# modichirag/GSM-VI

Measured on AMD Instinct MI355X. Metric: GSM updates/sec at D=1024,B=32 (dense-cov gsm_update, fp64), higher is better.
Workload: dtype f64; 1 GPU; BASELINE configs[2]: D=1024 dense-cov Gaussian target, B=32, one GSM update per step; D=1024, B=32, instances=21, ring_bytes=352321536, launch=hipGraph(90 x 21 updates/replay + 1 x 7), warmup_steps_run=28, parallelism=single GPU

## Files before the change

### gsm-vi_amd/csrc/gsmvi_abi.hip

```cpp
#include <hip/hip_runtime.h>

#include <cstdio>
#include <cstdlib>
#include <cstring>
#include <string>

#include "../../include/gsmvi_hip.h"
#include "../../include/gsmvi_hip_debug.h"

void gsmvi_launch_panel_partial(hipStream_t st, hipEvent_t* ev, int MT, dim3 grid, int D, int ncols, int nrows,
                                const double* A, int lda, const double* shift, double alpha, const double* M,
                                int ldm, double* Pp, int chunks_per_wg, int a_vec_ok);
void gsmvi_launch_panel_finish(hipStream_t st, hipEvent_t* ev, int D, int nrows, int KC, const double* Pp,
                               const double* addvec, double* Out, int ldo, int ncols_out);
void gsmvi_launch_gsm_scalars(hipStream_t st, hipEvent_t* ev, int D, int B, int KC, const double* X, int ldx,
                              const double* G, int ldg, const double* mu0, const double* Pp, double* rec,
                              int ldrec);
size_t gsmvi_cov_update_lds_bytes(int SB);
hipError_t gsmvi_cov_update_prepare();
hipError_t gsmvi_bam_prepare();
hipError_t gsmvi_batched_prepare();
hipError_t gsmvi_bam_batched_prepare();
hipError_t gsmvi_psis_batched_prepare();
hipError_t gsmvi_psis_loo_batched_prepare();
// ... 4 lines not shown
                          const double* M, int ldm, int mrows, double* Pp, int* kc_out);
void gsmvi_launch_commit(hipStream_t st, int D, const int* info, const double* mu_new, const double* S_new,
                         int lds_new, double* mu, double* S, int lds, int* n_reverts);
void gsmvi_launch_panel_fast(hipStream_t st, hipEvent_t* ev, int MT, dim3 grid, int D, int nrows, const double* A,
                             int lda, const double* shift, double alpha, const double* M, int ldm, double* Pp,
                             int chunks_per_wg, int ncols, unsigned long long* stamps, double* Out, int ldo,
                             const double* addvec, const struct gsmvi_panel_extras* px);
bool gsmvi_launch_gsm_scalars_fast(hipStream_t st, hipEvent_t* ev, int D, int B, int KC, const double* X, int ldx,
                                   const double* G, int ldg, const double* mu0, const double* Pp, double* rec,
                                   int ldrec, int nt, unsigned long long* stamps);
bool gsmvi_launch_gsm_cov_sym(hipStream_t st, hipEvent_t* ev, int D, int B, const double* rec, int ldrec,
                              const double* mu0, const double* S0, int lds0, double* S, int lds, double* mu_out,
                              int dbg, unsigned long long* stamps, int num_cu);
void gsmvi_launch_panel_fast_part(hipStream_t st, hipEvent_t* ev, dim3 grid, int D, int B, const double* G, int ldg,
                                  const double* S0, int lds0, double* Pp, int chunks_per_wg, const double* X, int ldx,
                                  const double* mu0, double* Qg, double* Qm, int chw, unsigned long long* stamps);
void gsmvi_launch_gsm_cov_sym_slabs(hipStream_t st, hipEvent_t* ev, int D, int B, const struct gsm_slab_src& fs, const double* mu0,
                                    const double* S0, int lds0, double* S, int lds, double* mu_out, int kct, bool fold,
                                    unsigned long long* stamps);
int gsmvi_cov_sym_pairs(int nt);
int gsmvi_panel_fast_chunk(int MT);
int gsmvi_potrf_impl(struct gsmvi_ctx* ctx, hipStream_t st, int D, const double* S, int lds, double* R, int ldr,
                     int* info_dev);
int gsmvi_gram_impl(hipStream_t st, int D, const double* F, int ldf, double* C, int ldc, double shift, const double* shift_dev);
int gsmvi_whiten_impl(hipStream_t st, int D, int nrows, const double* R, int ldr, const double* X, int ldx,
                      const double* mu, double* Z, int ldz, double* logdiag);
int gsmvi_factor_impl(struct gsmvi_ctx* ctx, hipStream_t st, int D, int B, const double* Z, int ldz, const double* X,
                      int ldx, const double* G, int ldg, const double* mu0, const double* F0, int ldf0, double* mu,
                      double* F, int ldf, int* info_dev, int* n_reverts_dev);
int gsmvi_factor_local_impl(struct gsmvi_ctx* ctx, hipStream_t st, int D, int Bl, const double* Z, int ldz,
                            const double* X, int ldx, const double* G, int ldg, const double* mu0, const double* F0,
                            int ldf0, double* rec, int ldrec);
int gsmvi_factor_apply_impl(struct gsmvi_ctx* ctx, hipStream_t st, int D, int B, const double* Z, int ldz,
                            const double* rec, int ldrec, const double* mu0, const double* F0, int ldf0, double* mu,
// ... 230 lines not shown
    else if (!strcmp(name, "wide")) ctx->tune_wide = value;
    else if (!strcmp(name, "wide_kc")) ctx->tune_wide_kc = value;
    else if (!strcmp(name, "fork_min_D")) ctx->tune_fork_min_D = value;
    else if (!strcmp(name, "gram_mt")) ctx->tune_gram_mt = value > 0 ? value : 4;
    else if (!strcmp(name, "bam_full")) ctx->tune_bam_full = value;
    else if (!strcmp(name, "bam_kenq")) ctx->tune_bam_kenq = value;
    else if (!strcmp(name, "bam_hint_slack")) ctx->tune_bam_hint_slack = value;
    else if (!strcmp(name, "rider_direct_max_D")) ctx->tune_rider_direct_max_D = value;
    else if (!strcmp(name, "chain_pair")) ctx->tune_chain_pair = value;
    else if (!strcmp(name, "bam_batched_pad")) ctx->tune_bam_batched_pad = value;
    else if (!strcmp(name, "lowrank_kp")) ctx->tune_lowrank_kp = value;
    else if (!strcmp(name, "bam_basis")) ctx->tune_bam_basis = value;
    else if (!strcmp(name, "scalars_nt")) ctx->tune_scalars_nt = value;
    else if (!strcmp(name, "gsm_two_launch")) ctx->tune_gsm_two_launch = value;
    else if (!strcmp(name, "cov_fold_diag")) ctx->tune_cov_fold_diag = value;
    else if (!strcmp(name, "cov_dbg")) ctx->tune_cov_dbg = value;
    else if (!strcmp(name, "timeline")) {
        if (value && !ctx->stamps) {
            HIP_TRY(hipMalloc(reinterpret_cast<void**>(&ctx->stamps), GSMVI_STAMP_WORDS * sizeof(unsigned long long)));
            HIP_TRY(hipMemset(ctx->stamps, 0, GSMVI_STAMP_WORDS * sizeof(unsigned long long)));
        }
        ctx->tune_timeline = value;
    }
    else {
        gsmvi_set_error("%s: unknown tuning knob %s", __func__, name);
        return GSMVI_ERR_BAD_ARG;
    }
    return GSMVI_OK;
}

// ... 278 lines not shown
        *chw_out = 512;
    }
    return true;
}

static int gsm_two_launch(gsmvi_ctx* ctx, hipStream_t hs, int D, int B, int cpw, int kc, int chw, const double* X, int ldx,
                          const double* G, int ldg, const double* mu0, const double* S0, int lds0, double* mu, double* S,
                          int lds) {
    const int strips = D / 16;
    double* Qg = ctx->sg;
    double* Qm = Qg + (size_t)B * kc * strips;
    ctx->px = gsmvi_panel_extras();
    ctx->px_used = 1;
    hipEvent_t* ev0 = ctx->stage_events(0);
    ctx->ev_valid[1] = 0;
    gsmvi_launch_panel_fast_part(hs, ev0, dim3(strips, kc, chw == 512 ? B / 16 : 1), D, B, G, ldg, S0, lds0, ctx->pp, cpw, X, ldx, mu0, Qg, Qm, chw,
                                 ctx->timeline_stamps(0));
    ctx->path |= GSMVI_PATH_PANEL_FAST | (chw == 512 ? GSMVI_PATH_PANEL_CHUNK512 : 0u);
    int st = check_launch("k_panel_fast(partials)");
    if (st != GSMVI_OK) return st;
    gsm_slab_src fs;
    fs.X = X;
    fs.ldx = ldx;
    fs.Pp = ctx->pp;
    fs.Qg = Qg;
    fs.Qm = Qm;
    fs.KC = kc;
    fs.strips = strips;
    const bool fold = ctx->tune_cov_fold_diag >= 2 || (ctx->tune_cov_fold_diag == 1 && gsmvi_cov_sym_pairs(D / 32) >= ctx->num_cu);
    gsmvi_launch_gsm_cov_sym_slabs(hs, ctx->stage_events(2), D, B, fs, mu0, S0, lds0, S, lds, mu, chw == 512 ? 2 : 4, fold,
                                   ctx->timeline_stamps(2));
    ctx->path |= GSMVI_PATH_COV_SYM | GSMVI_PATH_GSM_TWO_LAUNCH | (fold ? GSMVI_PATH_COV_FOLD_DIAG : 0u);
    return check_launch("k_gsm_cov_sym(slabs)");
}

int gsmvi_gsm_update_f64(gsmvi_ctx* ctx, void* stream, int D, int B, const double* X, int ldx, const double* G,
                         int ldg, const double* mu0, const double* S0, int lds0, double* mu, double* S, int lds) {
    int st = check_common(ctx, D, B, __func__);
    if (st != GSMVI_OK) return st;
    BAD_ARG(!X || !G || !mu0 || !S0 || !mu || !S, "NULL array");
    BAD_ARG(ldx < D || ldg < D || lds0 < D || lds < D, "leading dimension smaller than D");
    BAD_ARG(S == S0 || mu == mu0, "outputs must not alias inputs");
    hipStream_t hs = reinterpret_cast<hipStream_t>(stream);
    const int ldrec = 3 * D + (D & 1);
    int cpw2 = 0, kc2 = 0, chw2 = 0;
    if (gsm_two_launch_gate(ctx, D, B, X, ldx, G, ldg, mu0, S0, lds0, S, lds, &cpw2, &kc2, &chw2))
        return gsm_two_launch(ctx, hs, D, B, cpw2, kc2, chw2, X, ldx, G, ldg, mu0, S0, lds0, mu, S, lds);
// ... 294 lines not shown
```

### gsm-vi_amd/csrc/gsmvi_ctx.h

```cpp
#pragma once
#include <hip/hip_runtime.h>
#include <cstddef>

#define GSMVI_MAX_KC 8
#define GSMVI_FACTOR_NMAX 256
#define GSMVI_STAMP_WORDS (4 * 4096)

struct gsmvi_panel_extras {
    const double* msl = nullptr;
    int kcm = 0;
    size_t mstride = 0;
    int ldsl = 0, msplit = 0;
    double* mfin = nullptr;
    int ldfin = 0;
    const double* sj_src = nullptr;
    int sj_kc = 0;
    size_t sj_stride = 0;
    int sj_len = 0;
    double* sj_dst = nullptr;
    int rd_on = 0, rd_n = 0, rd_B = 0, rd_kcg = 0, rd_jmode = 0;
    const double* rd_Gp = nullptr;
    double *rd_Kmat = nullptr, *rd_coef = nullptr;
    int* rd_bad = nullptr;
    unsigned long long* rd_stamps = nullptr;
// ... 52 lines not shown
    double* pp = nullptr;
    double* sg = nullptr;
    double *fo_Rt = nullptr, *fo_Tm = nullptr, *fo_Fs = nullptr;
    double* small = nullptr;
    int* ints = nullptr;
    double* gram_slabs = nullptr;
    int tune_panel_kc = 0;
    int tune_update_sb = 0;
    int tune_cov_dbg = 0;
    int tune_timeline = 0;
    unsigned long long* stamps = nullptr;
    int tune_direct_out = 1;
    int tune_scalars_nt = 0;
    int tune_no_fast = 0;
    int tune_cov_fold_diag = 1;
    int tune_gsm_two_launch = 1;
    int* bam_hint_host = nullptr;
    int tune_bam_kenq = 0;
    int tune_bam_hint_slack = 1;
    int tune_rider_direct_max_D = 2048;
    int tune_bam_full = 0;
    int tune_lowrank_kp = 0;
    int tune_bam_batched_pad = 1;
    int tune_chain_pair = 1;
    gsmf_bam_mean bam_mean = {nullptr, nullptr, {0.0, nullptr}};
    int bam_mean_done = 0;
    const double* chain_r11 = nullptr;
    const double* chain_w11 = nullptr;
    const double* reg_dev = nullptr;
    int tune_bam_basis = 1;
// ... 50 lines not shown
```

### gsm-vi_amd/csrc/gsmvi_fast.hip

```cpp
#include "gsmvi_common.h"
#include "gsmvi_ctx.h"
#include "gsmvi_small16.h"
#include <hip/hip_ext.h>

#define GSMVI_LAUNCH(kern, grid, block, shmem, st, ev, ...)                                         \
    do {                                                                                           \
        if (ev)                                                                                    \
            hipExtLaunchKernelGGL(kern, grid, block, shmem, st, (ev)[0], (ev)[1], 0, __VA_ARGS__); \
        else                                                                                       \
            hipLaunchKernelGGL(kern, grid, block, shmem, st, __VA_ARGS__);                         \
    } while (0)

template <int MT, bool HAS_SHIFT, int CHW, bool EXTRA, bool RIDER = false, bool RAG = false, bool PART = false>
__global__ __launch_bounds__(512) void k_panel_fast(int D, int nrows, const double* __restrict__ A, int lda,
                                                    const double* __restrict__ shift, double alpha,
                                                    const double* __restrict__ M, int ldm,
                                                    double* Pp, int chunks_per_wg, int ncols,
                                                    unsigned long long* __restrict__ stamps, double* __restrict__ Out,
                                                    int ldo, const double* __restrict__ addvec, gsmvi_panel_extras px) {
#define PSTAMP(k)                                                                                              \
    do {                                                                                                       \
        const unsigned wg_ = (blockIdx.z * gridDim.y + blockIdx.y) * gridDim.x + blockIdx.x;                   \
        if (stamps && threadIdx.x == 0 && wg_ < GSMVI_STAMP_WG)                                                \
            stamps[(size_t)wg_ * 8 + (k)] = __builtin_amdgcn_s_memrealtime();                                  \
    } while (0)
    PSTAMP(0);
    constexpr int LDG = CHW + 2;
    constexpr int NR = 16 * MT;
// ... 7 lines not shown
    if (RIDER && blockIdx.x == gridDim.x - 1) {
        if (blockIdx.y == 0 && blockIdx.z == 0)
            gsmf_small16_body(As, px.rd_n, px.rd_B, px.rd_Gp, px.rd_kcg, px.rd_Kmat, px.rd_coef, px.rd_bad, px.rd_stamps,
                              px.rd_jmode, px.rd_prior, px.rd_Pi, px.rd_R11, px.rd_W11);
        return;
    }
    const int tid = threadIdx.x, w = tid >> 6, l = tid & 63, c = l & 15, ks = l >> 4;
    const int jx = blockIdx.x * 16 + c;
    const int j = (RAG && jx >= ncols) ? ncols - 1 : jx;
    const int r0 = blockIdx.z * NR;

    v4d acc[MT];
#pragma unroll
    for (int mt = 0; mt < MT; ++mt) acc[mt] = (v4d){0.0, 0.0, 0.0, 0.0};
    static_assert(!PART || (MT <= 2 && !RAG && !RIDER && !HAS_SHIFT), "partial dots: one pass of the store loop, on the grid");
    double pq_g = 0.0, pq_x = 0.0, pq_m = 0.0;

    for (int ch = 0; ch < chunks_per_wg; ++ch) {
        const int cbase = (blockIdx.y * chunks_per_wg + ch) * CHW;
        if (cbase >= D) break;
        const int wbase = cbase + w * RW;
        const bool wave_in = wbase < D;
        v2d ga[UPT];
        v2d gs[UPT];
        unsigned okbits = 0;
#pragma unroll
        for (int q = 0; q < UPT; ++q) {
            const int u = q * 512 + tid;
            const int row = u / U16, c16 = u % U16;
            const int grow = r0 + row;
            const int col = cbase + 2 * c16;
// ... 44 lines not shown
        } else if (!RAG || wbase + RW <= D) {
            const double* mp = M + (size_t)((wave_in ? wbase : 0) + ks) * ldm + j;
#pragma unroll
            for (int s = 0; s < NST; ++s) m[s] = mp[(size_t)(4 * s) * ldm];
        } else {
            const int rb = wave_in ? wbase : 0;
#pragma unroll
            for (int s = 0; s < NST; ++s) {
                const int r = rb + ks + 4 * s;
                m[s] = M[(size_t)(r < D ? r : D - 1) * ldm + j];
            }
        }
        if constexpr (PART) {
            const int prow = r0 + ((tid >> 4) & (NR - 1)), pcol = blockIdx.x * 16 + (tid & 15);
            pq_g = A[(size_t)prow * lda + pcol];
            pq_x = px.sj_src[(size_t)prow * px.sj_len + pcol];
            pq_m = px.msl[pcol];
        }
        __builtin_amdgcn_sched_barrier(0);
        if (ch > 0) __syncthreads();
#pragma unroll
        for (int q = 0; q < UPT; ++q) {
            const int u = q * 512 + tid;
            const int row = u / U16, c16 = u % U16;
            v2d v = ga[q];
            if (!((okbits >> q) & 1u)) v = HAS_SHIFT ? gs[q] : (v2d){0.0, 0.0};
            if (HAS_SHIFT) { v.x -= gs[q].x; v.y -= gs[q].y; }
            v.x *= alpha; v.y *= alpha;
            *reinterpret_cast<v2d*>(&As[row * LDG + 2 * c16]) = v;
        }
        __syncthreads();
        PSTAMP(1);
// ... 20 lines not shown
#pragma unroll
        for (int r = 0; r < 4; ++r) red[(w * NR + 16 * mt + ks + 4 * r) * 17 + c] = acc[mt][r];
    __syncthreads();
    for (int idx = tid; idx < NR * 16; idx += 512) {
        const int rr = idx >> 4, cc = idx & 15;
        const int row = r0 + rr;
        if (row < nrows && (!RAG || (int)blockIdx.x * 16 + cc < ncols)) {
            double s = 0.0;
#pragma unroll
            for (int ww = 0; ww < 8; ww += 2) s += red[(ww * NR + rr) * 17 + cc] + red[((ww + 1) * NR + rr) * 17 + cc];
            if (Out == nullptr) Pp[((size_t)blockIdx.y * nrows + row) * ncols + blockIdx.x * 16 + cc] = s;
            else Out[(size_t)row * ldo + blockIdx.x * 16 + cc] = s + (addvec ? addvec[blockIdx.x * 16 + cc] : 0.0);
            if constexpr (PART) {
                const double pg = row16_sum(pq_g * s);
                if (cc == 0) px.sj_dst[((size_t)row * gridDim.y + blockIdx.y) * gridDim.x + blockIdx.x] = pg;
                if (blockIdx.y == 0) {
                    const double pm = row16_sum((pq_m - pq_x) * pq_g);
                    if (cc == 0) px.mfin[(size_t)row * gridDim.x + blockIdx.x] = pm;
                }
            }
        }
    }
    if (EXTRA && px.sj_src != nullptr) {
        const int nwg = gridDim.x * gridDim.y * gridDim.z;
        const int wg = (blockIdx.z * gridDim.y + blockIdx.y) * gridDim.x + blockIdx.x;
        const int per = (px.sj_len + nwg - 1) / nwg;
        const int i_end = (wg + 1) * per < px.sj_len ? (wg + 1) * per : px.sj_len;
        for (int i = wg * per + tid; i < i_end; i += (int)blockDim.x) {
            double t[GSMVI_MAX_KC];
#pragma unroll
            for (int q = 0; q < GSMVI_MAX_KC; ++q) t[q] = px.sj_src[(size_t)(q < px.sj_kc ? q : px.sj_kc - 1) * px.sj_stride + i];
            double a = 0.0;
#pragma unroll
            for (int q = 0; q < GSMVI_MAX_KC; ++q) a += (q < px.sj_kc) ? t[q] : 0.0;
// ... 159 lines not shown
    for (int e = 0; e < EPT; ++e) {
        const int i = tid + NT * e;
        if (i < D) {
            const double dmu = beta * ((sg[e] - dd[e]) - c * dd[e]);
            rb[i] = dd[e];
            rb[D + i] = dd[e] + dmu;
            rb[2 * D + i] = dmu;
        }
    }
    if (stamps) {
        asm volatile("s_waitcnt vmcnt(0)" ::: "memory");
        if (threadIdx.x == 0) stamps[(size_t)blockIdx.x * 8 + 3] = __builtin_amdgcn_s_memrealtime();
    }
}

template <int SB, bool RAG, bool FROM_SLABS = false, int KCT = 4, bool FOLD = false>
__global__ __launch_bounds__(512) __attribute__((amdgpu_waves_per_eu(FROM_SLABS ? 4 : 2))) void k_gsm_cov_sym(int D, int B, double invB, const double* __restrict__ rec, int ldrec,
                                                     const double* __restrict__ mu0,
                                                     const double* __restrict__ S0, int lds0,
                                                     double* __restrict__ S, int lds,
                                                     double* __restrict__ mu_out, int dbg,
                                                     unsigned long long* __restrict__ stamps, gsm_slab_src fs) {
    static_assert(!FOLD || FROM_SLABS, "folded diagonal tiles: the two-launch form only");
#define STAMP(k)                                                                          \
    do {                                                                                  \
        if (stamps && threadIdx.x == 0) stamps[(size_t)blockIdx.x * 8 + (k)] = __builtin_amdgcn_s_memrealtime(); \
    } while (0)
    if (blockIdx.x >= GSMVI_STAMP_WG) stamps = nullptr;
    STAMP(0);
    constexpr int RS = 48;
    constexpr int NPASS = (SB > 32) ? SB / 32 : 1;
    constexpr int SBP = SB / NPASS;
    constexpr int TILE = SBP * RS;
    constexpr int NU = SB * 16;
    constexpr int UPT = (6 * NU) / 512;
    static_assert((6 * NU) % 512 == 0, "tile units must divide over 512 threads");
    __shared__ __attribute__((aligned(16))) double smem[6 * TILE >= 2 * 32 * 33 ? 6 * TILE : 2 * 32 * 33];

// ... 18 lines not shown
        const int k = blockIdx.x - n_two;
        ti = ((nt & 1) ? 0 : 1) + 2 * k;
        tj0 = ti;
        two = false;
    }
    const bool diag = (tj0 == ti);
    const int I0 = ti * 32, J0 = tj0 * 32;
    const int tid = threadIdx.x, w = tid >> 6, l = tid & 63, c = l & 15, ks = l >> 4;
    const int t = w >> 2;
    const int wr = (w >> 1) & 1, wc = w & 1;
    const bool mine = (t == 0) || two;

    const int Jt = J0 + 32 * ((t == 1 && two) ? 1 : 0);
    const int tl = tid & 255;
    v2d s0v[2];
#pragma unroll
    for (int q = 0; q < 2; ++q) {
        const int unit = q * 256 + tl, i = unit >> 4, j2 = unit & 15;
        const int gr = (RAG && I0 + i >= D) ? D - 1 : I0 + i, gc = (RAG && Jt + 2 * j2 >= D) ? D - 2 : Jt + 2 * j2;
        s0v[q] = (dbg & 2) ? (v2d){1.0, 1.0} : *reinterpret_cast<const v2d*>(S0 + (size_t)gr * lds0 + gc);
    }
    const int X0 = (fold == 2) ? J0 + 32 : I0;
    v2d s0x = {0.0, 0.0};
    if constexpr (FOLD) {
        if (fold) s0x = *reinterpret_cast<const v2d*>(S0 + (size_t)(X0 + (tid >> 4)) * lds0 + X0 + 2 * (tid & 15));
    }
    __builtin_amdgcn_sched_barrier(0);
    v2d stg[UPT];
    double dmu_part = 0.0;
    v2d dmuI = {0.0, 0.0};
    v2d dmuX = {0.0, 0.0};
    if constexpr (FROM_SLABS) {
        static_assert(!RAG && NPASS == 1 && 512 % NU == 0, "two-launch form: B == SB in {16, 32}, on the grid");
        static_assert(KCT == 2 || KCT == 4, "slab count of the two-launch form");
        constexpr int NQG = 2 * KCT;
        const int u = tid & (NU - 1), b = u >> 4, ln = u & 15, c2 = 2 * ln;
        const bool st_d = (NU == 512) || tid < NU, st_e = (NU == 512) || tid >= NU;
        const int nqg = (fs.KC * fs.strips) >> 1, nqm = fs.strips >> 1;
        auto ld16 = [](const double* base, unsigned byte_off) {
            return *reinterpret_cast<const v2d*>(reinterpret_cast<const char*>(base) + byte_off);
        };
        const unsigned qg0 = (unsigned)(b * nqg) * 16u, qm0 = (unsigned)(b * nqm) * 16u;
        v2d qg[NQG], qm[2];
#pragma unroll
        for (int k = 0; k < NQG; ++k) qg[k] = ld16(fs.Qg, qg0 + 16u * (unsigned)(ln + 16 * k < nqg ? ln + 16 * k : nqg - 1));
#pragma unroll
        for (int k = 0; k < 2; ++k) qm[k] = ld16(fs.Qm, qm0 + 16u * (unsigned)(ln + 16 * k < nqm ? ln + 16 * k : nqm - 1));
        const int col[3] = {I0 + c2, J0 + c2, J0 + 32 + c2};
        const size_t slab = (size_t)B * D;
        v2d xv[3], m0[3], sl[3][KCT];
        auto load_block = [&](int cb) {
            xv[cb] = *reinterpret_cast<const v2d*>(fs.X + (size_t)b * fs.ldx + col[cb]);
            m0[cb] = ld16(mu0, 8u * (unsigned)col[cb]);
#pragma unroll
            for (int kc = 0; kc < KCT; ++kc)
                sl[cb][kc] = *reinterpret_cast<const v2d*>(fs.Pp + (size_t)(KCT == 2 ? kc : (kc < fs.KC ? kc : fs.KC - 1)) * slab + (size_t)b * D + col[cb]);
        };
        load_block(0);
        load_block(1);
        if constexpr (KCT == 2) {
            if (two) load_block(2);
        }
        double gs = 0.0, ms = 0.0;
#pragma unroll
        for (int k = 0; k < NQG; ++k) {
            const bool in = ln + 16 * k < nqg;
            gs += in ? qg[k].x : 0.0;
            gs += in ? qg[k].y : 0.0;
        }
#pragma unroll
        for (int k = 0; k < 2; ++k) {
            const bool in = ln + 16 * k < nqm;
            ms += in ? qm[k].x : 0.0;
            ms += in ? qm[k].y : 0.0;
        }
        if constexpr (KCT == 4) {
            asm volatile("" : "+v"(gs), "+v"(ms) : : "memory");
            if (two) load_block(2);
        }
        const double gSg = row16_sum(gs), mv = row16_sum(ms);
        const double rho = 0.5 * sqrt(1.0 + 4.0 * (gSg + mv * mv)) - 0.5;
        const double den = 1.0 + rho + mv;
        double beta = 1.0 / (1.0 + rho), c = (gSg - mv) / den;
        if (stamps) { asm volatile("s_waitcnt vmcnt(0)" ::: "memory"); STAMP(1); }
#pragma unroll
        for (int cb = 0; cb < 3; ++cb)
            if (cb < 2 || two) {
                v2d sg = {0.0, 0.0}, dd, dm, ee;
                if constexpr (KCT == 2) {
                    if (cb == 0) asm volatile("" : "+v"(beta), "+v"(c), "+v"(xv[0]), "+v"(m0[0]), "+v"(sl[0][0]), "+v"(sl[0][1]));
                    else asm volatile("" : "+v"(xv[cb]), "+v"(m0[cb]), "+v"(sl[cb][0]), "+v"(sl[cb][1]));
                }
                if constexpr (KCT == 2) {
                    sg.x = sl[cb][0].x + sl[cb][1].x;
                    sg.y = sl[cb][0].y + sl[cb][1].y;
                } else {
#pragma unroll
                    for (int kc = 0; kc < 4; ++kc) {
                        sg.x += (kc < fs.KC) ? sl[cb][kc].x : 0.0;
// ... 30 lines not shown
            for (int k = 0; k < SB / 8; ++k) {
                const int b = (tid >> 5) + 8 * k, ci = I0 + (tid & 31);
                dv[k] = rec[(size_t)((RAG && b >= B) ? B - 1 : b) * ldrec + 2 * D + ((RAG && ci >= D) ? D - 1 : ci)];
            }
#pragma unroll
            for (int k = 0; k < SB / 8; ++k) dmu_part += (!RAG || (tid >> 5) + 8 * k < B) ? dv[k] : 0.0;
        }
    }
    if (!FROM_SLABS && stamps) { asm volatile("s_waitcnt vmcnt(0)" ::: "memory"); STAMP(1); }

    constexpr int NS = SBP / 4;
    v4d accd = {0.0, 0.0, 0.0, 0.0}, acce = {0.0, 0.0, 0.0, 0.0};
    v4d xaccd = {0.0, 0.0, 0.0, 0.0}, xacce = {0.0, 0.0, 0.0, 0.0};
#pragma unroll
    for (int pass = 0; pass < NPASS; ++pass) {
        if (pass > 0) __syncthreads();
        if constexpr (!FROM_SLABS) {
#pragma unroll
            for (int q = 0; q < UPT; ++q) {
                const int g = q * 512 + tid;
                const int tile = g / NU, u = g % NU;
                const int b = u >> 4;
                if (b / SBP == pass && (two || tile < 4))
                    *reinterpret_cast<v2d*>(smem + tile * TILE + (b % SBP) * RS + 2 * (u & 15)) = (!RAG || b < B) ? stg[q] : (v2d){0.0, 0.0};
            }
        }
        __syncthreads();
        if (pass == 0) STAMP(2);
        double ad[NS], ae[NS], bd[NS], be[NS];
        if (mine) {
            const double* adp = smem + ks * RS + 16 * wr + c;
            const double* aep = adp + TILE;
            const double* bdp = smem + (2 + 2 * t) * TILE + ks * RS + 16 * wc + c;
            const double* bep = bdp + TILE;
#pragma unroll
            for (int s = 0; s < NS; ++s) {
                ad[s] = adp[4 * s * RS];
                ae[s] = aep[4 * s * RS];
                bd[s] = bdp[4 * s * RS];
                be[s] = bep[4 * s * RS];
            }
        }
// ... 10 lines not shown
#pragma unroll
                for (int s = 0; s < NS; ++s) {
                    ad[s] = xdp[4 * s * RS + 16 * wr];
                    ae[s] = xdp[TILE + 4 * s * RS + 16 * wr];
                    bd[s] = xdp[4 * s * RS + 16 * wc];
                    be[s] = xdp[TILE + 4 * s * RS + 16 * wc];
                }
#pragma unroll
                for (int s = 0; s < NS; ++s) {
                    xaccd = GSMVI_MFMA_F64(ad[s], bd[s], xaccd);
                    xacce = GSMVI_MFMA_F64(ae[s], be[s], xacce);
                }
            }
        }
    }
    __syncthreads();
    double* LW = smem + t * 32 * 33;
    if (mine) {
#pragma unroll
        for (int r = 0; r < 4; ++r) LW[(16 * wr + ks + 4 * r) * 33 + 16 * wc + c] = (accd[r] - acce[r]) * invB;
    }
    constexpr int LXO = 2 * 32 * 33, MUO = 3 * 32 * 33;
    if constexpr (FOLD) {
        static_assert(!FOLD || MUO + SB * 32 + 256 <= 6 * TILE, "third LW buffer and the dmu tile inside the staged tiles");
        if (fold && t == 0) {
#pragma unroll
            for (int r = 0; r < 4; ++r) smem[LXO + (16 * wr + ks + 4 * r) * 33 + 16 * wc + c] = (xaccd[r] - xacce[r]) * invB;
        }
        if (fold && tid < NU) *reinterpret_cast<v2d*>(smem + MUO + (tid >> 4) * 32 + 2 * (tid & 15)) = dmuX;
    }
    if (stamps) STAMP(3);
    __syncthreads();
    if constexpr (FOLD) {
        if (fold && tid < 256) {
            double part = 0.0;
#pragma unroll
            for (int k = 0; k < SB / 8; ++k) part += smem[MUO + ((tid >> 5) + 8 * k) * 32 + (tid & 31)];
            smem[MUO + SB * 32 + tid] = part;
        }
    }
    if (mine) {
#pragma unroll
        for (int q = 0; q < 2; ++q) {
            const int unit = q * 256 + tl, i = unit >> 4, j2 = unit & 15;
            v2d wv2;
            wv2.x = s0v[q].x + LW[i * 33 + 2 * j2];
            wv2.y = s0v[q].y + LW[i * 33 + 2 * j2 + 1];
            if (!RAG || (I0 + i < D && Jt + 2 * j2 < D)) *reinterpret_cast<v2d*>(S + (size_t)(I0 + i) * lds + Jt + 2 * j2) = wv2;
            LW[i * 33 + 2 * j2] = wv2.x;
            LW[i * 33 + 2 * j2 + 1] = wv2.y;
        }
    }
    const bool need = mine && !(t == 0 && diag) && !(dbg & 1);
    __syncthreads();
    if (need) {
#pragma unroll
        for (int q = 0; q < 2; ++q) {
            const int unit = q * 256 + tl, j = unit >> 4, i2 = unit & 15;
            v2d m2;
            m2.x = LW[(2 * i2) * 33 + j];
            m2.y = LW[(2 * i2 + 1) * 33 + j];
            if (!RAG || (Jt + j < D && I0 + 2 * i2 < D)) *reinterpret_cast<v2d*>(S + (size_t)(Jt + j) * lds + I0 + 2 * i2) = m2;
        }
    }
    if constexpr (FOLD) {
        if (fold) {
            if (tid < 32) {
                double s = 0.0;
#pragma unroll
                for (int q = 0; q < 8; ++q) s += smem[MUO + SB * 32 + q * 32 + tid];
                mu_out[X0 + tid] = mu0[X0 + tid] + s * invB;
            }
            const int i = tid >> 4, j2 = tid & 15;
            v2d wv2;
            wv2.x = s0x.x + smem[LXO + i * 33 + 2 * j2];
            wv2.y = s0x.y + smem[LXO + i * 33 + 2 * j2 + 1];
            *reinterpret_cast<v2d*>(S + (size_t)(X0 + i) * lds + X0 + 2 * j2) = wv2;
        }
    }
    if (diag) {
        __syncthreads();
        if constexpr (FROM_SLABS) {
            if (tid < NU) *reinterpret_cast<v2d*>(smem + (tid >> 4) * 32 + 2 * (tid & 15)) = dmuI;
            __syncthreads();
            if (tid < 256) {
#pragma unroll
                for (int k = 0; k < SB / 8; ++k) dmu_part += smem[((tid >> 5) + 8 * k) * 32 + (tid & 31)];
                smem[SB * 32 + tid] = dmu_part;
            }
        } else {
            if (tid < 256) smem[tid] = dmu_part;
        }
        __syncthreads();
        if (tid < 32) {
            double s = 0.0;
#pragma unroll
            for (int q = 0; q < 8; ++q) s += smem[(FROM_SLABS ? SB * 32 : 0) + q * 32 + tid];
            if (!RAG || I0 + tid < D) mu_out[I0 + tid] = mu0[I0 + tid] + s * invB;
        }
    }
    STAMP(4);
    if (stamps) { asm volatile("s_waitcnt vmcnt(0)" ::: "memory"); STAMP(5); }
#undef STAMP
}

template <int SB, bool RAG>
__global__ __launch_bounds__(512) void k_gsm_cov_sym_p(int D, int B, double invB, const double* __restrict__ rec, int ldrec,
                                                       const double* __restrict__ mu0,
                                                       const double* __restrict__ S0, int lds0,
                                                       double* __restrict__ S, int lds,
                                                       double* __restrict__ mu_out) {
#define LDS_BARRIER() asm volatile("s_waitcnt lgkmcnt(0)\n\ts_barrier" ::: "memory")
    constexpr int RS = 48;
    constexpr int NPASS = (SB > 32) ? SB / 32 : 1;
    constexpr int SBP = SB / NPASS;
    constexpr int TILE = SBP * RS;
    constexpr int NU = SB * 16;
    constexpr int UPT = (6 * NU) / 512;
// ... 359 lines not shown
    do {                                                                                \
        if (rag) { if (extra) PF(MTV, HS, CW, true, true); else PF(MTV, HS, CW, false, true); } \
        else { if (extra) PF(MTV, HS, CW, true, false); else PF(MTV, HS, CW, false, false); }   \
    } while (0)
    if (shift) {
        if (MT == 1) PFE(1, true, 256); else if (MT == 2) PFE(2, true, 256); else PFE(4, true, 128);
    } else {
        if (MT == 1) PFE(1, false, 256); else if (MT == 2) PFE(2, false, 256); else PFE(4, false, 128);
    }
#undef PFE
#undef PF
}

void gsmvi_launch_panel_fast_part(hipStream_t st, hipEvent_t* ev, dim3 grid, int D, int B, const double* G, int ldg,
                                  const double* S0, int lds0, double* Pp, int chunks_per_wg, const double* X, int ldx,
                                  const double* mu0, double* Qg, double* Qm, int chw, unsigned long long* stamps) {
    gsmvi_panel_extras px;
    px.sj_src = X;
    px.sj_len = ldx;
    px.msl = mu0;
    px.sj_dst = Qg;
    px.mfin = Qm;
#define PFQ(MTV, CW) GSMVI_LAUNCH((k_panel_fast<MTV, false, CW, false, false, false, true>), grid, dim3(512), 0, st, ev, D, B, G, ldg, \
                                  nullptr, 1.0, S0, lds0, Pp, chunks_per_wg, D, stamps, nullptr, 0, nullptr, px)
    if (chw == 512) PFQ(1, 512);
    else { if (B == 16) PFQ(1, 256); else PFQ(2, 256); }
#undef PFQ
}

int gsmvi_panel_fast_chunk(int MT) { return MT == 4 ? 128 : 256; }

bool gsmvi_launch_gsm_scalars_fast(hipStream_t st, hipEvent_t* ev, int D, int B, int KC, const double* X, int ldx,
                                   const double* G, int ldg, const double* mu0, const double* Pp, double* rec,
                                   int ldrec, int nt, unsigned long long* stamps) {
    if (nt != 256 && nt != 512 && nt != 1024) nt = 512;
    const int ept = (D + nt - 1) / nt;
#define SF(E, K, N)                                                                                              \
    GSMVI_LAUNCH((k_gsm_scalars_fast<E, K, N>), dim3(B), dim3(N), 0, st, ev, D, B, KC, X, ldx, G, ldg, mu0, Pp, rec, \
                 ldrec, stamps)
#define SFK(E, N) do { if (kct == 1) SF(E, 1, N); else if (kct == 2) SF(E, 2, N); else if (kct == 4) SF(E, 4, N); else SF(E, 8, N); } while (0)
// ... 51 lines not shown
        }
    } else {
        switch (SB) {
            case 16: CS(16, false); break;
            case 32: CS(32, false); break;
            case 64: CS(64, false); break;
            default: CS(128, false); break;
        }
    }
#undef CS
    return true;
}

void gsmvi_launch_gsm_cov_sym_slabs(hipStream_t st, hipEvent_t* ev, int D, int B, const gsm_slab_src& fs, const double* mu0,
                                    const double* S0, int lds0, double* S, int lds, double* mu_out, int kct, bool fold,
                                    unsigned long long* stamps) {
    const dim3 grid(fold ? gsmvi_cov_sym_pairs(D / 32) : cov_sym_grid(D / 32));
    const double invB = 1.0 / (double)B;
#define CSS(SBV, KV, FV)                                                                                                  \
    GSMVI_LAUNCH((k_gsm_cov_sym<SBV, false, true, KV, FV>), grid, dim3(512), 0, st, ev, D, B, invB, nullptr, 0, mu0, S0, lds0, S, lds, mu_out, \
                 0, stamps, fs)
#define CSF(SBV, KV) do { if (fold) CSS(SBV, KV, true); else CSS(SBV, KV, false); } while (0)
    if (kct == 2) { if (B == 16) CSF(16, 2); else CSF(32, 2); }
    else { if (B == 16) CSF(16, 4); else CSF(32, 4); }
#undef CSF
#undef CSS
}
```

### gsm-vi_amd/engine.py

```python
import ctypes as C

import numpy as np
import torch

from . import _lib


def _require_gpu():
    if not torch.cuda.is_available():
        raise RuntimeError("gsmvi_amd needs an AMD GPU visible to torch (torch.cuda.is_available() is False); "
                           "there is no CPU fallback.")


def _unheld_entry(pool):
    import sys
    for e in pool:
        if sys.getrefcount(e[1]) <= 2:
            return e
    return None


def _device_index(device):
    if device is None:
        return torch.cuda.current_device()
# ... 401 lines not shown
        n, D = X.shape
        self._ensure(D, max(self._max_B, 1))
        Z = self.empty(n, D)
        ld = self.empty(1)
        self._call("gsmvi_whiten_rows_f64", D, n, *self._mat(R, "R"), *self._mat(X, "X"),
                   self._vec(mu, "mu") if mu is not None else None, *self._mat(Z, "Z"), _ptr(ld))
        return Z, ld

    PATH_BITS = {"panel_fast": 0x1, "panel_wide": 0x2, "panel_generic": 0x4, "panel_t_fast": 0x8, "panel_t_generic": 0x10,
                 "scalars_fast": 0x20, "scalars_generic": 0x40, "cov_sym": 0x80, "cov_generic": 0x100, "fupd_fast": 0x200,
                 "fupd_generic": 0x400, "lowrank_fast": 0x800, "lowrank_generic": 0x1000, "batched": 0x2000,
                 "batched_bam": 0x4000, "batched_kl": 0x8000, "batched_advi": 0x10000, "batched_target": 0x20000,
                 "batched_lbfgs": 0x40000, "batched_laplace": 0x80000, "batched_predict": 0x100000,
                 "batched_psis": 0x200000, "batched_loo": 0x400000, "gsm_two_launch": 0x800000,
                 "batched_softmax": 0x1000000, "panel_chunk512": 0x2000000, "batched_pathfinder": 0x4000000,
                 "cov_fold_diag": 0x8000000, "batched_softmax_laplace": 0x10000000}
    PATH_GENERIC_MASK = 0x4 | 0x10 | 0x40 | 0x100 | 0x400 | 0x1000

    def last_path(self, reset=True):
        self._any_ctx()
        bits = C.c_uint(0)
        self._call_ctx("gsmvi_last_path", C.byref(bits), int(bool(reset)))
        return {k for k, v in self.PATH_BITS.items() if bits.value & v}

    def bam_reg_source(self, word):
        self._any_ctx()
        self._reg_word = word
        self._call_ctx("gsmvi_bam_set_reg_source", _ptr(word))

    def set_profiling(self, on):
        self._any_ctx()
# ... 520 lines not shown
```

### include/gsmvi_hip.h

```cpp
#ifndef GSMVI_HIP_H
#define GSMVI_HIP_H

#include <stddef.h>
#include <stdint.h>

#ifdef __cplusplus
extern "C" {
#endif
#pragma GCC visibility push(default)

#define GSMVI_ABI_VERSION 1

typedef enum gsmvi_status {
    GSMVI_OK = 0,
    GSMVI_ERR_BAD_ARG = 1,
    GSMVI_ERR_HIP = 2,
    GSMVI_ERR_NO_DEVICE = 3,
    GSMVI_ERR_WORKSPACE = 4,
    GSMVI_ERR_UNSUPPORTED = 5
} gsmvi_status;

typedef struct gsmvi_ctx gsmvi_ctx;

int gsmvi_abi_version(void);
// ... 81 lines not shown
#define GSMVI_PATH_BATCHED_BAM 0x4000u
#define GSMVI_PATH_BATCHED_KL 0x8000u
#define GSMVI_PATH_BATCHED_ADVI 0x10000u
#define GSMVI_PATH_BATCHED_TARGET 0x20000u
#define GSMVI_PATH_BATCHED_LBFGS 0x40000u
#define GSMVI_PATH_BATCHED_LAPLACE 0x80000u
#define GSMVI_PATH_BATCHED_PREDICT 0x100000u
#define GSMVI_PATH_BATCHED_PSIS 0x200000u
#define GSMVI_PATH_BATCHED_LOO 0x400000u
#define GSMVI_PATH_GSM_TWO_LAUNCH 0x800000u
#define GSMVI_PATH_BATCHED_SOFTMAX 0x1000000u
#define GSMVI_PATH_PANEL_CHUNK512 0x2000000u
#define GSMVI_PATH_BATCHED_PATHFINDER 0x4000000u
#define GSMVI_PATH_COV_FOLD_DIAG 0x8000000u
#define GSMVI_PATH_BATCHED_SOFTMAX_LAPLACE 0x10000000u
#define GSMVI_PATH_GENERIC_MASK (0x0004u | 0x0010u | 0x0040u | 0x0100u | 0x0400u | 0x1000u)
int gsmvi_last_path(gsmvi_ctx* ctx, unsigned* bits, int reset);

int gsmvi_bam_set_reg_source(gsmvi_ctx* ctx, const double* reg_dev);

int gsmvi_gaussian_score_f64(gsmvi_ctx* ctx, void* stream, int D, int B,
                             const double* X, int ldx, const double* m,
                             const double* P, int ldp, double* G, int ldg);

int gsmvi_gsm_update_batched_f64(gsmvi_ctx* ctx, void* stream, int64_t K, int D, int B, const double* X, const double* G,
                                 const double* mu0, const double* S0, double* mu, double* S);

int gsmvi_gsm_fit_init_batched_f64(gsmvi_ctx* ctx, void* stream, int64_t K, int D, int B, const double* mean, const double* cov,
                                   double* R, int* info_dev, const uint64_t* seeds_dev, double* X);

// ... 165 lines not shown
```

Baseline: 63050 updates/s.

## Add S0-late loads, buffer-store write-through, and whole-sample Qm options to GSM two-launch path

Adds three tuning options to the two-launch dense-cov GSM update. Only the buffer-resource store path for the S output is on by default; the other two default off. One option defers the S0 tile loads until after the slab loads, using lgkmcnt-only barriers so those loads overlap the LDS work. Another has a subset of panel workgroups compute the full per-sample mean projection, so the cov kernel reads one scalar instead of reducing partials. The buffer-store path drops bounds checks and may change cache write behaviour, but adds template variants and relies on the byte offset fitting in 31 bits.

```diff
diff --git a/gsm-vi_amd/csrc/gsmvi_abi.hip b/gsm-vi_amd/csrc/gsmvi_abi.hip
--- a/gsm-vi_amd/csrc/gsmvi_abi.hip
+++ b/gsm-vi_amd/csrc/gsmvi_abi.hip
@@ -42,10 +42,10 @@
                               int dbg, unsigned long long* stamps, int num_cu);
 void gsmvi_launch_panel_fast_part(hipStream_t st, hipEvent_t* ev, dim3 grid, int D, int B, const double* G, int ldg,
                                   const double* S0, int lds0, double* Pp, int chunks_per_wg, const double* X, int ldx,
-                                  const double* mu0, double* Qg, double* Qm, int chw, unsigned long long* stamps);
+                                  const double* mu0, double* Qg, double* Qm, int chw, bool qm_whole, unsigned long long* stamps);
 void gsmvi_launch_gsm_cov_sym_slabs(hipStream_t st, hipEvent_t* ev, int D, int B, const struct gsm_slab_src& fs, const double* mu0,
                                     const double* S0, int lds0, double* S, int lds, double* mu_out, int kct, bool fold,
-                                    unsigned long long* stamps);
+                                    bool s0_last, bool store_wt, bool qm_whole, unsigned long long* stamps);
 int gsmvi_cov_sym_pairs(int nt);
 int gsmvi_panel_fast_chunk(int MT);
 int gsmvi_potrf_impl(struct gsmvi_ctx* ctx, hipStream_t st, int D, const double* S, int lds, double* R, int ldr,
@@ -306,6 +306,9 @@
     else if (!strcmp(name, "scalars_nt")) ctx->tune_scalars_nt = value;
     else if (!strcmp(name, "gsm_two_launch")) ctx->tune_gsm_two_launch = value;
     else if (!strcmp(name, "cov_fold_diag")) ctx->tune_cov_fold_diag = value;
+    else if (!strcmp(name, "cov_s0_last")) ctx->tune_cov_s0_last = value;
+    else if (!strcmp(name, "cov_store_wt")) ctx->tune_cov_store_wt = value;
+    else if (!strcmp(name, "panel_qm_whole")) ctx->tune_panel_qm_whole = value;
     else if (!strcmp(name, "cov_dbg")) ctx->tune_cov_dbg = value;
     else if (!strcmp(name, "timeline")) {
         if (value && !ctx->stamps) {
@@ -614,9 +617,10 @@
     ctx->px_used = 1;
     hipEvent_t* ev0 = ctx->stage_events(0);
     ctx->ev_valid[1] = 0;
+    const bool qm_whole = chw == 512 && D == 1024 && ctx->tune_panel_qm_whole != 0;
     gsmvi_launch_panel_fast_part(hs, ev0, dim3(strips, kc, chw == 512 ? B / 16 : 1), D, B, G, ldg, S0, lds0, ctx->pp, cpw, X, ldx, mu0, Qg, Qm, chw,
-                                 ctx->timeline_stamps(0));
-    ctx->path |= GSMVI_PATH_PANEL_FAST | (chw == 512 ? GSMVI_PATH_PANEL_CHUNK512 : 0u);
+                                 qm_whole, ctx->timeline_stamps(0));
+    ctx->path |= GSMVI_PATH_PANEL_FAST | (chw == 512 ? GSMVI_PATH_PANEL_CHUNK512 : 0u) | (qm_whole ? GSMVI_PATH_PANEL_QM_WHOLE : 0u);
     int st = check_launch("k_panel_fast(partials)");
     if (st != GSMVI_OK) return st;
     gsm_slab_src fs;
@@ -628,9 +632,12 @@
     fs.KC = kc;
     fs.strips = strips;
     const bool fold = ctx->tune_cov_fold_diag >= 2 || (ctx->tune_cov_fold_diag == 1 && gsmvi_cov_sym_pairs(D / 32) >= ctx->num_cu);
+    const bool s0_last = chw == 512 && ctx->tune_cov_s0_last != 0;
+    const bool store_wt = chw == 512 && ctx->tune_cov_store_wt != 0 && (size_t)D * (size_t)lds * sizeof(double) < ((size_t)1 << 31);
     gsmvi_launch_gsm_cov_sym_slabs(hs, ctx->stage_events(2), D, B, fs, mu0, S0, lds0, S, lds, mu, chw == 512 ? 2 : 4, fold,
-                                   ctx->timeline_stamps(2));
-    ctx->path |= GSMVI_PATH_COV_SYM | GSMVI_PATH_GSM_TWO_LAUNCH | (fold ? GSMVI_PATH_COV_FOLD_DIAG : 0u);
+                                   s0_last, store_wt, qm_whole, ctx->timeline_stamps(2));
+    ctx->path |= GSMVI_PATH_COV_SYM | GSMVI_PATH_GSM_TWO_LAUNCH | (fold ? GSMVI_PATH_COV_FOLD_DIAG : 0u) |
+                 (s0_last ? GSMVI_PATH_COV_S0_LAST : 0u) | (store_wt ? GSMVI_PATH_COV_STORE_WT : 0u);
     return check_launch("k_gsm_cov_sym(slabs)");
 }
 
diff --git a/gsm-vi_amd/csrc/gsmvi_ctx.h b/gsm-vi_amd/csrc/gsmvi_ctx.h
--- a/gsm-vi_amd/csrc/gsmvi_ctx.h
+++ b/gsm-vi_amd/csrc/gsmvi_ctx.h
@@ -90,6 +90,9 @@
     int tune_scalars_nt = 0;
     int tune_no_fast = 0;
     int tune_cov_fold_diag = 1;
+    int tune_cov_s0_last = 0;
+    int tune_cov_store_wt = 1;
+    int tune_panel_qm_whole = 0;
     int tune_gsm_two_launch = 1;
     int* bam_hint_host = nullptr;
     int tune_bam_kenq = 0;
diff --git a/gsm-vi_amd/csrc/gsmvi_fast.hip b/gsm-vi_amd/csrc/gsmvi_fast.hip
--- a/gsm-vi_amd/csrc/gsmvi_fast.hip
+++ b/gsm-vi_amd/csrc/gsmvi_fast.hip
@@ -11,7 +11,7 @@
             hipLaunchKernelGGL(kern, grid, block, shmem, st, __VA_ARGS__);                         \
     } while (0)
 
-template <int MT, bool HAS_SHIFT, int CHW, bool EXTRA, bool RIDER = false, bool RAG = false, bool PART = false>
+template <int MT, bool HAS_SHIFT, int CHW, bool EXTRA, bool RIDER = false, bool RAG = false, bool PART = false, bool QMW = false>
 __global__ __launch_bounds__(512) void k_panel_fast(int D, int nrows, const double* __restrict__ A, int lda,
                                                     const double* __restrict__ shift, double alpha,
                                                     const double* __restrict__ M, int ldm,
@@ -49,7 +49,9 @@
 #pragma unroll
     for (int mt = 0; mt < MT; ++mt) acc[mt] = (v4d){0.0, 0.0, 0.0, 0.0};
     static_assert(!PART || (MT <= 2 && !RAG && !RIDER && !HAS_SHIFT), "partial dots: one pass of the store loop, on the grid");
+    static_assert(!QMW || (PART && CHW == 512 && MT == 1), "whole-sample Qm: the 512-row-chunk product of the two-launch form");
     double pq_g = 0.0, pq_x = 0.0, pq_m = 0.0;
+    [[maybe_unused]] v2d wq_g, wq_x, wq_m;
 
     for (int ch = 0; ch < chunks_per_wg; ++ch) {
         const int cbase = (blockIdx.y * chunks_per_wg + ch) * CHW;
@@ -124,8 +126,15 @@
         if constexpr (PART) {
             const int prow = r0 + ((tid >> 4) & (NR - 1)), pcol = blockIdx.x * 16 + (tid & 15);
             pq_g = A[(size_t)prow * lda + pcol];
-            pq_x = px.sj_src[(size_t)prow * px.sj_len + pcol];
-            pq_m = px.msl[pcol];
+            if constexpr (!QMW) {
+                pq_x = px.sj_src[(size_t)prow * px.sj_len + pcol];
+                pq_m = px.msl[pcol];
+            } else if (blockIdx.y == 1 && blockIdx.x < 16) {
+                const int qm_b = 16 * blockIdx.z + blockIdx.x, qm_c = 2 * tid < D ? 2 * tid : 0;
+                wq_g = *reinterpret_cast<const v2d*>(A + (size_t)qm_b * lda + qm_c);
+                wq_x = *reinterpret_cast<const v2d*>(px.sj_src + (size_t)qm_b * px.sj_len + qm_c);
+                wq_m = *reinterpret_cast<const v2d*>(px.msl + qm_c);
+            }
         }
         __builtin_amdgcn_sched_barrier(0);
         if (ch > 0) __syncthreads();
@@ -176,10 +185,26 @@
             if constexpr (PART) {
                 const double pg = row16_sum(pq_g * s);
                 if (cc == 0) px.sj_dst[((size_t)row * gridDim.y + blockIdx.y) * gridDim.x + blockIdx.x] = pg;
-                if (blockIdx.y == 0) {
+                if (!QMW && blockIdx.y == 0) {
                     const double pm = row16_sum((pq_m - pq_x) * pq_g);
                     if (cc == 0) px.mfin[(size_t)row * gridDim.x + blockIdx.x] = pm;
                 }
+            }
+        }
+    }
+    if constexpr (QMW) {
+        if (blockIdx.y == 1 && blockIdx.x < 16) {
+            const int qm_b = 16 * blockIdx.z + blockIdx.x;
+            const double pr = 2 * tid < D ? (wq_m.x - wq_x.x) * wq_g.x + (wq_m.y - wq_x.y) * wq_g.y : 0.0;
+            const double rs = row16_sum(pr);
+            __syncthreads();
+            if ((tid & 15) == 0) red[tid >> 4] = rs;
+            __syncthreads();
+            if (tid == 0) {
+                double s = 0.0;
+#pragma unroll
+                for (int i = 0; i < 32; ++i) s += red[i];
+                px.mfin[qm_b] = s;
             }
         }
     }
@@ -369,7 +394,8 @@
     }
 }
 
-template <int SB, bool RAG, bool FROM_SLABS = false, int KCT = 4, bool FOLD = false>
+typedef unsigned int v4u __attribute__((ext_vector_type(4)));
+template <int SB, bool RAG, bool FROM_SLABS = false, int KCT = 4, bool FOLD = false, bool S0L = false, bool WT = false, bool QMW = false>
 __global__ __launch_bounds__(512) __attribute__((amdgpu_waves_per_eu(FROM_SLABS ? 4 : 2))) void k_gsm_cov_sym(int D, int B, double invB, const double* __restrict__ rec, int ldrec,
                                                      const double* __restrict__ mu0,
                                                      const double* __restrict__ S0, int lds0,
@@ -377,6 +403,12 @@
                                                      double* __restrict__ mu_out, int dbg,
                                                      unsigned long long* __restrict__ stamps, gsm_slab_src fs) {
     static_assert(!FOLD || FROM_SLABS, "folded diagonal tiles: the two-launch form only");
+    static_assert(!(S0L || WT || QMW) || (FROM_SLABS && KCT == 2 && !RAG), "S0 last / write-through stores / whole-sample Qm: the two-slab two-launch form only, on the grid");
+#define PRE_W_BARRIER()                                                                   \
+    do {                                                                                  \
+        if constexpr (S0L) asm volatile("s_waitcnt lgkmcnt(0)\n\ts_barrier" ::: "memory"); \
+        else __syncthreads();                                                             \
+    } while (0)
 #define STAMP(k)                                                                          \
     do {                                                                                  \
         if (stamps && threadIdx.x == 0) stamps[(size_t)blockIdx.x * 8 + (k)] = __builtin_amdgcn_s_memrealtime(); \
@@ -425,18 +457,20 @@
     const int Jt = J0 + 32 * ((t == 1 && two) ? 1 : 0);
     const int tl = tid & 255;
     v2d s0v[2];
-#pragma unroll
-    for (int q = 0; q < 2; ++q) {
-        const int unit = q * 256 + tl, i = unit >> 4, j2 = unit & 15;
-        const int gr = (RAG && I0 + i >= D) ? D - 1 : I0 + i, gc = (RAG && Jt + 2 * j2 >= D) ? D - 2 : Jt + 2 * j2;
-        s0v[q] = (dbg & 2) ? (v2d){1.0, 1.0} : *reinterpret_cast<const v2d*>(S0 + (size_t)gr * lds0 + gc);
+    if constexpr (!S0L) {
+#pragma unroll
+        for (int q = 0; q < 2; ++q) {
+            const int unit = q * 256 + tl, i = unit >> 4, j2 = unit & 15;
+            const int gr = (RAG && I0 + i >= D) ? D - 1 : I0 + i, gc = (RAG && Jt + 2 * j2 >= D) ? D - 2 : Jt + 2 * j2;
+            s0v[q] = (dbg & 2) ? (v2d){1.0, 1.0} : *reinterpret_cast<const v2d*>(S0 + (size_t)gr * lds0 + gc);
+        }
     }
     const int X0 = (fold == 2) ? J0 + 32 : I0;
     v2d s0x = {0.0, 0.0};
-    if constexpr (FOLD) {
+    if constexpr (FOLD && !S0L) {
         if (fold) s0x = *reinterpret_cast<const v2d*>(S0 + (size_t)(X0 + (tid >> 4)) * lds0 + X0 + 2 * (tid & 15));
     }
-    __builtin_amdgcn_sched_barrier(0);
+    if constexpr (!S0L) __builtin_amdgcn_sched_barrier(0);
     v2d stg[UPT];
     double dmu_part = 0.0;
     v2d dmuI = {0.0, 0.0};
@@ -455,8 +489,12 @@
         v2d qg[NQG], qm[2];
 #pragma unroll
         for (int k = 0; k < NQG; ++k) qg[k] = ld16(fs.Qg, qg0 + 16u * (unsigned)(ln + 16 * k < nqg ? ln + 16 * k : nqg - 1));
-#pragma unroll
-        for (int k = 0; k < 2; ++k) qm[k] = ld16(fs.Qm, qm0 + 16u * (unsigned)(ln + 16 * k < nqm ? ln + 16 * k : nqm - 1));
+        [[maybe_unused]] double mvq = 0.0;
+        if constexpr (QMW) mvq = fs.Qm[b];
+        else {
+#pragma unroll
+            for (int k = 0; k < 2; ++k) qm[k] = ld16(fs.Qm, qm0 + 16u * (unsigned)(ln + 16 * k < nqm ? ln + 16 * k : nqm - 1));
+        }
         const int col[3] = {I0 + c2, J0 + c2, J0 + 32 + c2};
         const size_t slab = (size_t)B * D;
         v2d xv[3], m0[3], sl[3][KCT];
@@ -472,6 +510,19 @@
         if constexpr (KCT == 2) {
             if (two) load_block(2);
         }
+        if constexpr (S0L) {
+            __builtin_amdgcn_sched_barrier(0);
+#pragma unroll
+            for (int q = 0; q < 2; ++q) {
+                const int unit = q * 256 + tl;
+                s0v[q] = *reinterpret_cast<const v2d*>(S0 + (size_t)(I0 + (unit >> 4)) * lds0 + Jt + 2 * (unit & 15));
+            }
+            if constexpr (FOLD) {
+                const int xr = fold ? X0 + (tid >> 4) : I0 + ((256 + tl) >> 4), xc = fold ? X0 + 2 * (tid & 15) : Jt + 2 * (tl & 15);
+                s0x = *reinterpret_cast<const v2d*>(S0 + (size_t)xr * lds0 + xc);
+            }
+            __builtin_amdgcn_sched_barrier(0);
+        }
         double gs = 0.0, ms = 0.0;
 #pragma unroll
         for (int k = 0; k < NQG; ++k) {
@@ -479,21 +530,31 @@
             gs += in ? qg[k].x : 0.0;
             gs += in ? qg[k].y : 0.0;
         }
-#pragma unroll
-        for (int k = 0; k < 2; ++k) {
-            const bool in = ln + 16 * k < nqm;
-            ms += in ? qm[k].x : 0.0;
-            ms += in ? qm[k].y : 0.0;
+        if constexpr (!QMW) {
+#pragma unroll
+            for (int k = 0; k < 2; ++k) {
+                const bool in = ln + 16 * k < nqm;
+                ms += in ? qm[k].x : 0.0;
+                ms += in ? qm[k].y : 0.0;
+            }
         }
         if constexpr (KCT == 4) {
             asm volatile("" : "+v"(gs), "+v"(ms) : : "memory");
             if (two) load_block(2);
         }
-        const double gSg = row16_sum(gs), mv = row16_sum(ms);
+        const double gSg = row16_sum(gs);
+        double mv;
+        if constexpr (QMW) mv = mvq;
+        else mv = row16_sum(ms);
         const double rho = 0.5 * sqrt(1.0 + 4.0 * (gSg + mv * mv)) - 0.5;
         const double den = 1.0 + rho + mv;
         double beta = 1.0 / (1.0 + rho), c = (gSg - mv) / den;
-        if (stamps) { asm volatile("s_waitcnt vmcnt(0)" ::: "memory"); STAMP(1); }
+        if (stamps) {
+            if constexpr (!S0L) asm volatile("s_waitcnt vmcnt(0)" ::: "memory");
+            else if constexpr (FOLD) asm volatile("s_waitcnt vmcnt(3)" ::: "memory");
+            else asm volatile("s_waitcnt vmcnt(2)" ::: "memory");
+            STAMP(1);
+        }
 #pragma unroll
         for (int cb = 0; cb < 3; ++cb)
             if (cb < 2 || two) {
@@ -554,7 +615,7 @@
     v4d xaccd = {0.0, 0.0, 0.0, 0.0}, xacce = {0.0, 0.0, 0.0, 0.0};
 #pragma unroll
     for (int pass = 0; pass < NPASS; ++pass) {
-        if (pass > 0) __syncthreads();
+        if (pass > 0) PRE_W_BARRIER();
         if constexpr (!FROM_SLABS) {
 #pragma unroll
             for (int q = 0; q < UPT; ++q) {
@@ -565,7 +626,7 @@
                     *reinterpret_cast<v2d*>(smem + tile * TILE + (b % SBP) * RS + 2 * (u & 15)) = (!RAG || b < B) ? stg[q] : (v2d){0.0, 0.0};
             }
         }
-        __syncthreads();
+        PRE_W_BARRIER();
         if (pass == 0) STAMP(2);
         double ad[NS], ae[NS], bd[NS], be[NS];
         if (mine) {
@@ -606,7 +667,7 @@
             }
         }
     }
-    __syncthreads();
+    PRE_W_BARRIER();
     double* LW = smem + t * 32 * 33;
     if (mine) {
 #pragma unroll
@@ -622,7 +683,15 @@
         if (fold && tid < NU) *reinterpret_cast<v2d*>(smem + MUO + (tid >> 4) * 32 + 2 * (tid & 15)) = dmuX;
     }
     if (stamps) STAMP(3);
-    __syncthreads();
+    PRE_W_BARRIER();
+    if constexpr (S0L) {
+        if (stamps) { asm volatile("s_waitcnt vmcnt(0)" ::: "memory"); STAMP(6); }
+    }
+    [[maybe_unused]] __amdgpu_buffer_rsrc_t srs;
+    if constexpr (WT) srs = __builtin_amdgcn_make_buffer_rsrc(S, 0, (int)(((size_t)(D - 1) * lds + D) * sizeof(double)), 0x00020000);
+    [[maybe_unused]] auto store_wt = [&](size_t off, v2d v) {
+        __builtin_amdgcn_raw_buffer_store_b128(__builtin_bit_cast(v4u, v), srs, (int)(off * sizeof(double)), 0, 16);
+    };
     if constexpr (FOLD) {
         if (fold && tid < 256) {
             double part = 0.0;
@@ -638,7 +707,8 @@
             v2d wv2;
             wv2.x = s0v[q].x + LW[i * 33 + 2 * j2];
             wv2.y = s0v[q].y + LW[i * 33 + 2 * j2 + 1];
-            if (!RAG || (I0 + i < D && Jt + 2 * j2 < D)) *reinterpret_cast<v2d*>(S + (size_t)(I0 + i) * lds + Jt + 2 * j2) = wv2;
+            if constexpr (WT) store_wt((size_t)(I0 + i) * lds + Jt + 2 * j2, wv2);
+            else if (!RAG || (I0 + i < D && Jt + 2 * j2 < D)) *reinterpret_cast<v2d*>(S + (size_t)(I0 + i) * lds + Jt + 2 * j2) = wv2;
             LW[i * 33 + 2 * j2] = wv2.x;
             LW[i * 33 + 2 * j2 + 1] = wv2.y;
         }
@@ -652,7 +722,8 @@
             v2d m2;
             m2.x = LW[(2 * i2) * 33 + j];
             m2.y = LW[(2 * i2 + 1) * 33 + j];
-            if (!RAG || (Jt + j < D && I0 + 2 * i2 < D)) *reinterpret_cast<v2d*>(S + (size_t)(Jt + j) * lds + I0 + 2 * i2) = m2;
+            if constexpr (WT) store_wt((size_t)(Jt + j) * lds + I0 + 2 * i2, m2);
+            else if (!RAG || (Jt + j < D && I0 + 2 * i2 < D)) *reinterpret_cast<v2d*>(S + (size_t)(Jt + j) * lds + I0 + 2 * i2) = m2;
         }
     }
     if constexpr (FOLD) {
@@ -667,7 +738,8 @@
             v2d wv2;
             wv2.x = s0x.x + smem[LXO + i * 33 + 2 * j2];
             wv2.y = s0x.y + smem[LXO + i * 33 + 2 * j2 + 1];
-            *reinterpret_cast<v2d*>(S + (size_t)(X0 + i) * lds + X0 + 2 * j2) = wv2;
+            if constexpr (WT) store_wt((size_t)(X0 + i) * lds + X0 + 2 * j2, wv2);
+            else *reinterpret_cast<v2d*>(S + (size_t)(X0 + i) * lds + X0 + 2 * j2) = wv2;
         }
     }
     if (diag) {
@@ -694,6 +766,7 @@
     STAMP(4);
     if (stamps) { asm volatile("s_waitcnt vmcnt(0)" ::: "memory"); STAMP(5); }
 #undef STAMP
+#undef PRE_W_BARRIER
 }
 
 template <int SB, bool RAG>
@@ -1083,7 +1156,7 @@
 
 void gsmvi_launch_panel_fast_part(hipStream_t st, hipEvent_t* ev, dim3 grid, int D, int B, const double* G, int ldg,
                                   const double* S0, int lds0, double* Pp, int chunks_per_wg, const double* X, int ldx,
-                                  const double* mu0, double* Qg, double* Qm, int chw, unsigned long long* stamps) {
+                                  const double* mu0, double* Qg, double* Qm, int chw, bool qm_whole, unsigned long long* stamps) {
     gsmvi_panel_extras px;
     px.sj_src = X;
     px.sj_len = ldx;
@@ -1092,7 +1165,10 @@
     px.mfin = Qm;
 #define PFQ(MTV, CW) GSMVI_LAUNCH((k_panel_fast<MTV, false, CW, false, false, false, true>), grid, dim3(512), 0, st, ev, D, B, G, ldg, \
                                   nullptr, 1.0, S0, lds0, Pp, chunks_per_wg, D, stamps, nullptr, 0, nullptr, px)
-    if (chw == 512) PFQ(1, 512);
+    if (chw == 512 && qm_whole)
+        GSMVI_LAUNCH((k_panel_fast<1, false, 512, false, false, false, true, true>), grid, dim3(512), 0, st, ev, D, B, G, ldg, nullptr, 1.0, S0,
+                     lds0, Pp, chunks_per_wg, D, stamps, nullptr, 0, nullptr, px);
+    else if (chw == 512) PFQ(1, 512);
     else { if (B == 16) PFQ(1, 256); else PFQ(2, 256); }
 #undef PFQ
 }
@@ -1174,15 +1250,25 @@
 
 void gsmvi_launch_gsm_cov_sym_slabs(hipStream_t st, hipEvent_t* ev, int D, int B, const gsm_slab_src& fs, const double* mu0,
                                     const double* S0, int lds0, double* S, int lds, double* mu_out, int kct, bool fold,
-                                    unsigned long long* stamps) {
+                                    bool s0_last, bool store_wt, bool qm_whole, unsigned long long* stamps) {
     const dim3 grid(fold ? gsmvi_cov_sym_pairs(D / 32) : cov_sym_grid(D / 32));
     const double invB = 1.0 / (double)B;
-#define CSS(SBV, KV, FV)                                                                                                  \
-    GSMVI_LAUNCH((k_gsm_cov_sym<SBV, false, true, KV, FV>), grid, dim3(512), 0, st, ev, D, B, invB, nullptr, 0, mu0, S0, lds0, S, lds, mu_out, \
-                 0, stamps, fs)
-#define CSF(SBV, KV) do { if (fold) CSS(SBV, KV, true); else CSS(SBV, KV, false); } while (0)
-    if (kct == 2) { if (B == 16) CSF(16, 2); else CSF(32, 2); }
-    else { if (B == 16) CSF(16, 4); else CSF(32, 4); }
+#define CSQ(SBV, KV, FV, LV, WV, QV)                                                                                      \
+    GSMVI_LAUNCH((k_gsm_cov_sym<SBV, false, true, KV, FV, LV, WV, QV>), grid, dim3(512), 0, st, ev, D, B, invB, nullptr, 0, mu0, S0, lds0, S, \
+                 lds, mu_out, 0, stamps, fs)
+#define CSS(SBV, KV, FV, LV, WV) do { if (KV == 2 && qm_whole) CSQ(SBV, 2, FV, LV, WV, true); else CSQ(SBV, KV, FV, LV, WV, false); } while (0)
+#define CSF(SBV, KV, LV, WV) do { if (fold) CSS(SBV, KV, true, LV, WV); else CSS(SBV, KV, false, LV, WV); } while (0)
+#define CSL(SBV)                                                                                                          \
+    do {                                                                                                                  \
+        if (s0_last && store_wt) CSF(SBV, 2, true, true);                                                                 \
+        else if (s0_last) CSF(SBV, 2, true, false);                                                                       \
+        else if (store_wt) CSF(SBV, 2, false, true);                                                                      \
+        else CSF(SBV, 2, false, false);                                                                                   \
+    } while (0)
+    if (kct == 2) { if (B == 16) CSL(16); else CSL(32); }
+    else { if (B == 16) CSF(16, 4, false, false); else CSF(32, 4, false, false); }
+#undef CSL
 #undef CSF
 #undef CSS
+#undef CSQ
 }
diff --git a/gsm-vi_amd/engine.py b/gsm-vi_amd/engine.py
--- a/gsm-vi_amd/engine.py
+++ b/gsm-vi_amd/engine.py
@@ -439,7 +439,8 @@
                  "batched_lbfgs": 0x40000, "batched_laplace": 0x80000, "batched_predict": 0x100000,
                  "batched_psis": 0x200000, "batched_loo": 0x400000, "gsm_two_launch": 0x800000,
                  "batched_softmax": 0x1000000, "panel_chunk512": 0x2000000, "batched_pathfinder": 0x4000000,
-                 "cov_fold_diag": 0x8000000, "batched_softmax_laplace": 0x10000000}
+                 "cov_fold_diag": 0x8000000, "batched_softmax_laplace": 0x10000000, "cov_s0_last": 0x20000000,
+                 "cov_store_wt": 0x40000000, "panel_qm_whole": 0x80000000}
     PATH_GENERIC_MASK = 0x4 | 0x10 | 0x40 | 0x100 | 0x400 | 0x1000
 
     def last_path(self, reset=True):
diff --git a/include/gsmvi_hip.h b/include/gsmvi_hip.h
--- a/include/gsmvi_hip.h
+++ b/include/gsmvi_hip.h
@@ -119,6 +119,9 @@
 #define GSMVI_PATH_BATCHED_PATHFINDER 0x4000000u
 #define GSMVI_PATH_COV_FOLD_DIAG 0x8000000u
 #define GSMVI_PATH_BATCHED_SOFTMAX_LAPLACE 0x10000000u
+#define GSMVI_PATH_COV_S0_LAST 0x20000000u
+#define GSMVI_PATH_COV_STORE_WT 0x40000000u
+#define GSMVI_PATH_PANEL_QM_WHOLE 0x80000000u
 #define GSMVI_PATH_GENERIC_MASK (0x0004u | 0x0010u | 0x0040u | 0x0100u | 0x0400u | 0x1000u)
 int gsmvi_last_path(gsmvi_ctx* ctx, unsigned* bits, int reset);
 
```

After: 66400 updates/s (median of 6 runs). 5.3% higher.
